# giolucasd/ssrl-vit-mae-jepa

Measured on AMD Instinct MI355X. Metric: images/sec pretrain step (fwd+bwd+opt), ViT-S/8 96px MAE, 1/2/4/8 MI355X, higher is better.
Workload: dtype bf16; 1 GPU; ViT-S/8 96px MAE (enc 384x12x6h, dec 192x2x6h, mask_ratio 0.75), batch 2000/GPU, full step; global_batch=2000, per_gpu_batch=2000, parallelism=dp1

## Files before the change

ssrl_vit_mae_jepa_amd/csrc/engine.hip:

```cpp
#include <string>
#include <vector>
#include <cmath>
#include <cstring>
#include <cstdlib>
#include <cstdint>
#include "kernels.h"

namespace mae {

static thread_local char g_err[1024] = "";
void set_error(const char* fmt, ...) {
  va_list ap;
  va_start(ap, fmt);
  vsnprintf(g_err, sizeof(g_err), fmt, ap);
  va_end(ap);
}
int hip_fail(hipError_t err, const char* what, const char* file, int line) {
  set_error("HIP error %d (%s) at %s:%d: %s", (int)err, hipGetErrorString(err), file, line, what);
  return 2;
}

struct ParamInfo {
  std::string name;
  int64_t offset = 0, numel = 0;
// ... 14 lines not shown
struct TimerSlot {
  std::vector<std::pair<hipEvent_t, hipEvent_t>> ev;
  size_t used = 0;
  double flops = 0, bytes = 0;
};

}

using namespace mae;

struct mae_engine {
  mae_config_t cfg;
  int act = MAE_F32;
  int D, depth, H, Dd, dd, Hd, P, L, G, C, img, p, mlp;
  int PO;
  std::vector<ParamInfo> params;
  int64_t arena_elems = 0, trainable_elems = 0, trans_elems = 0;
  int i_enc_mask, i_cls, i_pos, i_patch_w, i_patch_b, i_norm_w, i_norm_b;
  int i_dec_mask, i_dec_pos, i_de_w, i_de_b, i_dn_w, i_dn_b, i_pred_w, i_pred_b;
  std::vector<BlockRefs> enc, dec;
  bool timers_on = false;
  TimerSlot timers[TK_COUNT];
  PartialsTable ln_tab;
};

namespace mae {

static int add_param(mae_engine* e, const std::string& name, std::initializer_list<int64_t> shape, int flags) {
  ParamInfo pi;
  pi.name = name;
  pi.ndim = (int)shape.size();
  pi.numel = 1;
  int i = 0;
  for (int64_t s : shape) { pi.shape[i++] = s; pi.numel *= s; }
  pi.flags = flags;
  e->params.push_back(pi);
  return (int)e->params.size() - 1;
}

static BlockRefs add_block(mae_engine* e, const std::string& pfx, int d, int mlp) {
  const int T = MAE_PARAM_TRAINABLE, M = MAE_PARAM_TRAINABLE | MAE_PARAM_MATRIX;
  BlockRefs r;
  r.ln1_w = add_param(e, pfx + ".norm1.weight", {d}, T);
  r.ln1_b = add_param(e, pfx + ".norm1.bias", {d}, T);
  r.qkv_w = add_param(e, pfx + ".attn.qkv.weight", {3 * (int64_t)d, d}, M);
  r.qkv_b = add_param(e, pfx + ".attn.qkv.bias", {3 * (int64_t)d}, T);
// ... 2 lines not shown
  r.ln2_w = add_param(e, pfx + ".norm2.weight", {d}, T);
  r.ln2_b = add_param(e, pfx + ".norm2.bias", {d}, T);
  r.fc1_w = add_param(e, pfx + ".mlp.fc1.weight", {(int64_t)mlp * d, d}, M);
  r.fc1_b = add_param(e, pfx + ".mlp.fc1.bias", {(int64_t)mlp * d}, T);
  r.fc2_w = add_param(e, pfx + ".mlp.fc2.weight", {d, (int64_t)mlp * d}, M);
  r.fc2_b = add_param(e, pfx + ".mlp.fc2.bias", {d}, T);
  return r;
}

struct LayerBufs {
  int64_t x_mid, ln1, mean1, rstd1, qkv, lse, att, ln2, mean2, rstd2, fc1_pre, fc1_act;
};

struct Plan {
  int B, k, m;
  int dec_B, dec_T;
  int64_t Me, Md, Mp;
  int64_t keep32, mask32, inv, pred_rows;
  int64_t patchA;
  std::vector<int64_t> enc_x, dec_x;
  std::vector<LayerBufs> enc, dec;
  int64_t enc_norm, enc_mean, enc_rstd, xdec, dec_norm, dec_mean, dec_rstd, pred;
  int64_t branch_a, branch_b;
  int64_t dpred, d_decn, dres, dres_c, d_ln, d_att, d_qkv, d_hidden, d_xdec, dtok;
  int64_t ln_partial, ln_partial_stride, split_partial, wgrad_scratch, loss_scratch;
  int64_t total;
};

static Plan make_plan_ex(const mae_engine* e, int B, int k, int dec_B, int dec_T, int m_seq) {
  Plan pl;
  pl.B = B; pl.k = k; pl.m = m_seq;
  pl.dec_B = dec_B; pl.dec_T = dec_T;
  pl.Me = (int64_t)B * k; pl.Md = (int64_t)dec_B * dec_T; pl.Mp = (int64_t)dec_B * m_seq;
  const int64_t as = (int64_t)dtype_size(e->act);
  int64_t off = 0;
  auto take = [&](int64_t bytes) { const int64_t o = off; off += round_up(std::max<int64_t>(bytes, 4), 256); return o; };
  pl.keep32 = take(pl.Me * 4);
  pl.mask32 = take(pl.Mp * 4);
  pl.inv = take(pl.Md * 4);
  pl.pred_rows = take(pl.Mp * 4);
  pl.patchA = take(pl.Me * e->P * as);
  auto layers = [&](int n, int64_t M, int d, int heads, int T, std::vector<int64_t>& xs, std::vector<LayerBufs>& ls) {
    const int64_t seqs = M / std::max(T, 1);
    xs.resize(n + 1);
    ls.resize(n);
    xs[0] = take(M * d * 4);
    for (int i = 0; i < n; ++i) {
// ... 3 lines not shown
      b.lse = take(seqs * heads * T * 4);
      b.att = take(M * d * as);
      b.x_mid = take(M * d * 4);
      b.ln2 = take(M * d * as); b.mean2 = take(M * 4); b.rstd2 = take(M * 4);
      b.fc1_pre = take(M * e->mlp * d * as);
      b.fc1_act = take(M * e->mlp * d * as);
      xs[i + 1] = take(M * d * 4);
    }
  };
  layers(e->depth, pl.Me, e->D, e->H, k, pl.enc_x, pl.enc);
  pl.enc_norm = take(pl.Me * e->D * as); pl.enc_mean = take(pl.Me * 4); pl.enc_rstd = take(pl.Me * 4);
  pl.xdec = take(pl.Me * e->Dd * as);
  layers(e->dd, pl.Md, e->Dd, e->Hd, dec_T, pl.dec_x, pl.dec);
  pl.dec_norm = take(std::max<int64_t>(pl.Mp, 1) * e->Dd * as);
  pl.dec_mean = take(std::max<int64_t>(pl.Mp, 1) * 4); pl.dec_rstd = take(std::max<int64_t>(pl.Mp, 1) * 4);
  pl.pred = take(std::max<int64_t>(pl.Mp, 1) * e->PO * 4);
  const int64_t R = std::max(pl.Me * e->D, pl.Md * e->Dd);
  pl.branch_a = take(R * as);
  pl.branch_b = take(R * as);
  pl.dpred = take(std::max<int64_t>(pl.Mp, 1) * e->PO * as);
  pl.d_decn = take(std::max<int64_t>(pl.Mp, 1) * e->Dd * as);
  pl.dres = take(R * 4);
  pl.dres_c = take(R * as);
  pl.d_ln = take(R * as);
  pl.d_att = take(R * as);
  pl.d_qkv = take(3 * R * as);
  pl.d_hidden = take((int64_t)e->mlp * R * as);
  pl.d_xdec = take(pl.Me * e->Dd * as);
  pl.dtok = take(pl.Me * e->D * as);
  const int maxd = std::max(e->D, e->Dd);
  pl.ln_partial_stride = (int64_t)2 * LN_BWD_MAX_BLOCKS * maxd * 4;
  pl.ln_partial = take(pl.ln_partial_stride * std::min(2 * (e->depth + e->dd) + 2, (int)PartialsTable::MAX));
  pl.split_partial = take((int64_t)512 * maxd * 4);
  int64_t wg = 0;
  auto wgs = [&](int64_t M, int N, int K) { wg = std::max(wg, linear_wgrad_scratch_bytes(M, N, K)); };
  wgs(pl.Me, 3 * e->D, e->D); wgs(pl.Me, e->mlp * e->D, e->D); wgs(pl.Me, e->D, e->mlp * e->D); wgs(pl.Me, e->D, e->D);
  wgs(pl.Md, 3 * e->Dd, e->Dd); wgs(pl.Md, e->mlp * e->Dd, e->Dd); wgs(pl.Md, e->Dd, e->mlp * e->Dd); wgs(pl.Md, e->Dd, e->Dd);
  wgs(pl.Me, e->D, e->P); wgs(pl.Me, e->Dd, e->D); wgs(std::max<int64_t>(pl.Mp, 1), e->PO, e->Dd);
  auto wgp = [&](int64_t M, int d) {
    wg = std::max(wg, linear_wgrad_pair_scratch_bytes(M, d, e->mlp * d, e->mlp * d, d));
    wg = std::max(wg, linear_wgrad_pair_scratch_bytes(M, d, d, 3 * d, d));
  };
  wgp(pl.Me, e->D); wgp(pl.Md, e->Dd);
  pl.wgrad_scratch = take(wg);
  pl.loss_scratch = take(4096 * 4);
  pl.total = off;
// ... 58 lines not shown
  const int64_t side = mode == MAE_EPI_RESID ? 4 : (mode == MAE_EPI_MUL || mode == MAE_EPI_DGELU) ? os : 0;
  return (double)(M * K * as + (int64_t)N * K * as + M * N * (outs * os + side));
}

static int linear(const Ctx& c, const void* A, int wi, int bi, int64_t M, int N, int K, int mode, int out_dt, void* out, void* out2,
                  const void* aux) {
  mae_engine* e = c.e; hipStream_t s = c.s;
  Epi ep; ep.mode = mode; ep.bias = bi >= 0 ? c.P(bi) : nullptr; ep.aux = aux; ep.out = out; ep.out2 = out2; ep.out_dt = out_dt;
  RUN(TK_LINEAR, 2.0 * M * N * K, gemm_bytes(M, N, K, c.as, (int64_t)dtype_size(out_dt), mode), launch_linear_fwd(A, c.W(wi), M, N, K, c.act, ep, s));
  return 0;
}

static int dgrad(const Ctx& c, const void* dY, int wi, int64_t M, int N, int K, int mode, void* out, const void* aux) {
  mae_engine* e = c.e; hipStream_t s = c.s;
  Epi ep; ep.mode = mode; ep.aux = aux; ep.out = out; ep.out_dt = c.act;
  if (c.act == MAE_BF16) {
    RUN(TK_LINEAR, 2.0 * M * N * K, gemm_bytes(M, K, N, 2, 2, mode), launch_linear_fwd(dY, c.WT(wi), M, K, N, MAE_BF16, ep, s));
  } else {
    RUN(TK_LINEAR, 2.0 * M * N * K, gemm_bytes(M, K, N, 4, 4, mode), launch_linear_dgrad(dY, c.W(wi), M, N, K, MAE_F32, ep, s));
  }
  return 0;
}

static int wgrad(const Ctx& c, const Plan& pl, const void* dY, const void* A, int64_t M, int N, int K, int wi, int bi) {
  mae_engine* e = c.e; hipStream_t s = c.s;
  RUN(TK_WGRAD, 2.0 * M * N * K, (double)(M * (N + K) * c.as + (int64_t)N * K * 4),
      launch_linear_wgrad(dY, A, M, N, K, c.act, c.Gp(wi), bi >= 0 ? c.Gp(bi) : nullptr, c.buf<>(pl.wgrad_scratch), s));
  return 0;
}

static int wgrad_pair(const Ctx& c, const Plan& pl, int64_t M, const void* dY0, const void* A0, int N0, int K0, int w0, int b0,
                      const void* dY1, const void* A1, int N1, int K1, int w1, int b1) {
  mae_engine* e = c.e;
  hipStream_t s = c.s;
  RUN(TK_WGRAD, 2.0 * M * ((double)N0 * K0 + (double)N1 * K1),
      (double)(M * (int64_t)(N0 + K0 + N1 + K1) * c.as + ((int64_t)N0 * K0 + (int64_t)N1 * K1) * 4),
      launch_linear_wgrad_pair(dY0, A0, N0, K0, c.Gp(w0), c.Gp(b0), dY1, A1, N1, K1, c.Gp(w1), c.Gp(b1), M, c.act, c.buf<>(pl.wgrad_scratch), s));
  return 0;
}

static int ln_fwd(const Ctx& c, const float* x, const void* branch, float* x_sum, const int32_t* row_map, const float* gamma,
                  const float* beta, float eps, int64_t rows, int d, int y_dt, void* y, float* mean, float* rstd,
                  const float* image_scale = nullptr, int T = 0) {
  mae_engine* e = c.e; hipStream_t s = c.s;
  const int64_t ys = (int64_t)dtype_size(y_dt);
  RUN(TK_LN_FWD, 0, rows * d * (branch ? 8 + 2 * ys : 4 + ys),
      launch_layernorm_fwd(x, branch, x_sum, row_map, gamma, beta, eps, rows, d, y_dt, y, mean, rstd, s, image_scale, T));
  return 0;
}

static int ln_bwd(const Ctx& c, const Plan& pl, const void* dy, const float* x, const int32_t* row_map, int wi, int bi, const float* mean,
                  const float* rstd, int64_t rows, int d, int accumulate, const float* copy_scale = nullptr, int T = 0) {
  mae_engine* e = c.e; hipStream_t s = c.s;
  float* slot = c.buf<float>(pl.ln_partial + (int64_t)(e->ln_tab.n % PartialsTable::MAX) * pl.ln_partial_stride);
  RUN(TK_LN_BWD, 0, rows * d * (12 + 2 * c.as),
      launch_layernorm_bwd(dy, c.act, x, row_map, c.P(wi), mean, rstd, rows, d, accumulate, c.buf<float>(pl.dres), c.buf<>(pl.dres_c),
                           c.Gp(wi), c.Gp(bi), slot, s, &e->ln_tab, copy_scale, T));
  return 0;
}

static int block_forward(const Ctx& c, const Plan& pl, const BlockRefs& r, const LayerBufs& b, int64_t M, int d, int heads, int Bn, int T,
                         int64_t x_prev, bool add_prev, int64_t x_in, const float* scale_prev = nullptr, const float* scale_att = nullptr) {
  mae_engine* e = c.e; hipStream_t s = c.s;
  const int hd = d / heads, hid = e->mlp * d;
  const float eps = 1e-6f;
  MAE_TRY(ln_fwd(c, c.buf<float>(add_prev ? x_prev : x_in), add_prev ? c.buf<>(pl.branch_b) : nullptr, add_prev ? c.buf<float>(x_in) : nullptr,
                 nullptr, c.P(r.ln1_w), c.P(r.ln1_b), eps, M, d, c.act, c.buf<>(b.ln1), c.buf<float>(b.mean1), c.buf<float>(b.rstd1),
                 add_prev ? scale_prev : nullptr, T));
  MAE_TRY(linear(c, c.buf<>(b.ln1), r.qkv_w, r.qkv_b, M, 3 * d, d, MAE_EPI_NONE, c.act, c.buf<>(b.qkv), nullptr, nullptr));
  RUN(TK_ATTN_FWD, 4.0 * Bn * heads * (double)T * T * hd, M * 4 * d * c.as, launch_attention_fwd(c.buf<>(b.qkv), Bn, T, heads, hd, c.act, c.buf<>(b.att), c.buf<float>(b.lse), s));
  MAE_TRY(linear(c, c.buf<>(b.att), r.proj_w, r.proj_b, M, d, d, MAE_EPI_NONE, c.act, c.buf<>(pl.branch_a), nullptr, nullptr));
  MAE_TRY(ln_fwd(c, c.buf<float>(x_in), c.buf<>(pl.branch_a), c.buf<float>(b.x_mid), nullptr, c.P(r.ln2_w), c.P(r.ln2_b), eps, M, d, c.act,
                 c.buf<>(b.ln2), c.buf<float>(b.mean2), c.buf<float>(b.rstd2), scale_att, T));
  if (c.fwd_only)
    MAE_TRY(linear(c, c.buf<>(b.ln2), r.fc1_w, r.fc1_b, M, hid, d, MAE_EPI_GELU_ACT, c.act, c.buf<>(b.fc1_act), nullptr, nullptr));
  else
    MAE_TRY(linear(c, c.buf<>(b.ln2), r.fc1_w, r.fc1_b, M, hid, d, MAE_EPI_GELU_GRAD, c.act, c.buf<>(b.fc1_pre), c.buf<>(b.fc1_act), nullptr));
  MAE_TRY(linear(c, c.buf<>(b.fc1_act), r.fc2_w, r.fc2_b, M, d, hid, MAE_EPI_NONE, c.act, c.buf<>(pl.branch_b), nullptr, nullptr));
  return 0;
}

static int block_backward(const Ctx& c, const Plan& pl, const BlockRefs& r, const LayerBufs& b, int64_t M, int d, int heads, int Bn, int T,
                          int64_t x_in, const float* scale_prev = nullptr, const float* scale_att = nullptr) {
  mae_engine* e = c.e; hipStream_t s = c.s;
  const int hd = d / heads, hid = e->mlp * d;
  void* dres_c = c.buf<>(pl.dres_c);
  MAE_TRY(dgrad(c, dres_c, r.fc2_w, M, d, hid, MAE_EPI_MUL, c.buf<>(pl.d_hidden), c.buf<>(b.fc1_pre)));
  MAE_TRY(wgrad_pair(c, pl, M, dres_c, c.buf<>(b.fc1_act), d, hid, r.fc2_w, r.fc2_b, c.buf<>(pl.d_hidden), c.buf<>(b.ln2), hid, d, r.fc1_w, r.fc1_b));
  MAE_TRY(dgrad(c, c.buf<>(pl.d_hidden), r.fc1_w, M, hid, d, MAE_EPI_NONE, c.buf<>(pl.d_ln), nullptr));
  MAE_TRY(ln_bwd(c, pl, c.buf<>(pl.d_ln), c.buf<float>(b.x_mid), nullptr, r.ln2_w, r.ln2_b, c.buf<float>(b.mean2), c.buf<float>(b.rstd2), M, d, 1, scale_att, T));
  MAE_TRY(dgrad(c, dres_c, r.proj_w, M, d, d, MAE_EPI_NONE, c.buf<>(pl.d_att), nullptr));
  RUN(TK_ATTN_BWD, 10.0 * Bn * heads * (double)T * T * hd, M * 9 * d * c.as, launch_attention_bwd(c.buf<>(b.qkv), c.buf<>(b.att), c.buf<>(pl.d_att), c.buf<float>(b.lse), Bn, T, heads, hd, c.act, c.buf<>(pl.d_qkv), s));
  MAE_TRY(wgrad_pair(c, pl, M, dres_c, c.buf<>(b.att), d, d, r.proj_w, r.proj_b, c.buf<>(pl.d_qkv), c.buf<>(b.ln1), 3 * d, d, r.qkv_w, r.qkv_b));
  MAE_TRY(dgrad(c, c.buf<>(pl.d_qkv), r.qkv_w, M, 3 * d, d, MAE_EPI_NONE, c.buf<>(pl.d_ln), nullptr));
  MAE_TRY(ln_bwd(c, pl, c.buf<>(pl.d_ln), c.buf<float>(x_in), nullptr, r.ln1_w, r.ln1_b, c.buf<float>(b.mean1), c.buf<float>(b.rstd1), M, d, 1, scale_prev, T));
  return 0;
}

static bool batch_in_bound(const mae_engine* e, int B) {
  return (int64_t)B * e->L * std::max(3 * e->D, e->mlp * std::max(e->D, e->Dd)) < (1ll << 40);
}

static int check_common(const mae_engine* e, const void* params, const void* wcache, int B, const void* ws, const char* who) {
  MAE_REQUIRE(e, "%s: null engine", who);
  MAE_REQUIRE(params && ws, "%s: null params/workspace", who);
  MAE_REQUIRE(e->act == MAE_F32 || wcache, "%s: bf16 engine needs the weight cache", who);
  MAE_REQUIRE(batch_in_bound(e, B), "%s: batch too large", who);
  MAE_REQUIRE(((uintptr_t)ws & 255) == 0 && ((uintptr_t)params & 15) == 0, "%s: workspace must be 256-byte aligned, params 16-byte", who);
  return 0;
}

static int check_call(const mae_engine* e, const void* params, const void* wcache, int B, int k, const void* ws, int64_t ws_bytes,
                      Plan* pl, const char* who) {
  MAE_TRY(check_common(e, params, wcache, B, ws, who));
  MAE_REQUIRE(B > 0 && k >= 1 && k <= e->L, "%s: batch %d / num_keep %d out of range (L = %d)", who, B, k, e->L);
  *pl = make_plan(e, B, k);
  MAE_REQUIRE(ws_bytes >= pl->total, "%s: workspace too small (%lld < %lld bytes)", who, (long long)ws_bytes, (long long)pl->total);
// ... 39 lines not shown
static int forward_decoder_impl(const Ctx& c, const Plan& pl, float* x_pred_out, const JepaSeq* jp = nullptr) {
  mae_engine* e = c.e; hipStream_t s = c.s;
  MAE_REQUIRE(pl.m > 0, "forward_decoder: nothing is masked (num_keep == sequence_length)");
  MAE_TRY(linear(c, c.buf<>(pl.enc_norm), e->i_de_w, e->i_de_b, pl.Me, e->Dd, e->D, MAE_EPI_NONE, c.act, c.buf<>(pl.xdec), nullptr, nullptr));
  if (jp) {
    MAE_TRY(launch_build_tail_row_map(pl.dec_B, pl.dec_T, pl.m, c.buf<int32_t>(pl.pred_rows), s));
    RUN(TK_DATA, 0, pl.Md * e->Dd * 4 + pl.Me * e->Dd * c.as, launch_predictor_assemble(c.buf<>(pl.xdec), c.act, jp->ctx32, jp->tgt32, c.P(e->i_dec_mask), c.P(e->i_dec_pos), pl.B, pl.k, jp->nblk, pl.m, e->L, e->Dd, c.buf<float>(pl.dec_x[0]), s));
  } else {
    MAE_TRY(launch_build_inverse(c.buf<int32_t>(pl.keep32), pl.B, pl.k, e->L, c.buf<int32_t>(pl.inv), s));
    MAE_TRY(launch_build_row_map(c.buf<int32_t>(pl.mask32), pl.B, pl.m, e->L, c.buf<int32_t>(pl.pred_rows), s));
    RUN(TK_DATA, 0, pl.Md * e->Dd * 4 + pl.Me * e->Dd * c.as, launch_decoder_assemble(c.buf<>(pl.xdec), c.act, c.buf<int32_t>(pl.inv), c.P(e->i_dec_mask), c.P(e->i_dec_pos), pl.B, pl.k, e->L, e->Dd, c.buf<float>(pl.dec_x[0]), s));
  }
  for (int i = 0; i < e->dd; ++i)
    MAE_TRY(block_forward(c, pl, e->dec[i], pl.dec[i], pl.Md, e->Dd, e->Hd, pl.dec_B, pl.dec_T, i ? pl.dec[i - 1].x_mid : 0, i > 0, pl.dec_x[i]));
  MAE_TRY(ln_fwd(c, c.buf<float>(pl.dec[e->dd - 1].x_mid), c.buf<>(pl.branch_b), c.buf<float>(pl.dec_x[e->dd]), c.buf<int32_t>(pl.pred_rows),
                 c.P(e->i_dn_w), c.P(e->i_dn_b), 1e-6f, pl.Mp, e->Dd, c.act, c.buf<>(pl.dec_norm), c.buf<float>(pl.dec_mean), c.buf<float>(pl.dec_rstd)));
  MAE_TRY(linear(c, c.buf<>(pl.dec_norm), e->i_pred_w, e->i_pred_b, pl.Mp, e->PO, e->Dd, MAE_EPI_NONE, MAE_F32, x_pred_out ? (void*)x_pred_out : c.buf<>(pl.pred), nullptr, nullptr));
  return 0;
}

static int reach_point(const Ctx& c, int j) {
  mae_engine* e = c.e; hipStream_t s = c.s;
  if (!c.ready || !c.ready[j]) return 0;
  if (e->ln_tab.n > 0) {
    RUN(TK_LN_BWD, 0, 0, launch_sum_partials_many(e->ln_tab, s));
    e->ln_tab.n = 0;
  }
  MAE_HIP(hipEventRecord((hipEvent_t)c.ready[j], s));
  return 0;
}

static void backward_begin(const Ctx& c) { c.e->ln_tab.n = 0; }
static int backward_end(const Ctx& c) {
  mae_engine* e = c.e; hipStream_t s = c.s;
  if (e->ln_tab.n > 0) RUN(TK_LN_BWD, 0, 0, launch_sum_partials_many(e->ln_tab, s));
  e->ln_tab.n = 0;
  return 0;
}

static int backward_decoder_impl(const Ctx& c, const Plan& pl, const JepaSeq* jp = nullptr) {
  mae_engine* e = c.e; hipStream_t s = c.s;
  float* dres = c.buf<float>(pl.dres);
  MAE_TRY(wgrad(c, pl, c.buf<>(pl.dpred), c.buf<>(pl.dec_norm), pl.Mp, e->PO, e->Dd, e->i_pred_w, e->i_pred_b));
  MAE_TRY(dgrad(c, c.buf<>(pl.dpred), e->i_pred_w, pl.Mp, e->PO, e->Dd, MAE_EPI_NONE, c.buf<>(pl.d_decn), nullptr));
  RUN(TK_DATA, 0, (pl.Md - pl.Mp) * e->Dd * (4 + c.as), launch_zero_unpredicted_rows(jp ? nullptr : c.buf<int32_t>(pl.inv), pl.Md, pl.dec_T, pl.m, e->Dd, c.act, dres, c.buf<>(pl.dres_c), s));
  MAE_TRY(ln_bwd(c, pl, c.buf<>(pl.d_decn), c.buf<float>(pl.dec_x[e->dd]), c.buf<int32_t>(pl.pred_rows), e->i_dn_w, e->i_dn_b, c.buf<float>(pl.dec_mean),
                 c.buf<float>(pl.dec_rstd), pl.Mp, e->Dd, 0));
  for (int i = e->dd - 1; i >= 0; --i)
    MAE_TRY(block_backward(c, pl, e->dec[i], pl.dec[i], pl.Md, e->Dd, e->Hd, pl.dec_B, pl.dec_T, pl.dec_x[i]));
  if (jp)
    RUN(TK_DATA, 0, pl.Md * e->Dd * 4 + pl.Me * e->Dd * c.as, launch_predictor_assemble_bwd(dres, pl.B, pl.k, jp->nblk, pl.m, e->Dd, c.act, c.buf<>(pl.d_xdec), c.Gp(e->i_dec_mask), c.buf<float>(pl.split_partial), s));
  else
    RUN(TK_DATA, 0, pl.Md * e->Dd * 4 + pl.Me * e->Dd * c.as, launch_decoder_assemble_bwd(dres, c.buf<int32_t>(pl.inv), c.buf<int32_t>(pl.keep32), pl.B, pl.k, e->L, e->Dd, c.act, c.buf<>(pl.d_xdec), c.Gp(e->i_dec_mask), c.buf<float>(pl.split_partial), s));
  MAE_TRY(wgrad(c, pl, c.buf<>(pl.d_xdec), c.buf<>(pl.enc_norm), pl.Me, e->Dd, e->D, e->i_de_w, e->i_de_b));
  MAE_TRY(dgrad(c, c.buf<>(pl.d_xdec), e->i_de_w, pl.Me, e->Dd, e->D, MAE_EPI_NONE, c.buf<>(pl.d_ln), nullptr));
  return reach_point(c, 0);
}

static int backward_encoder_impl(const Ctx& c, const Plan& pl) {
  mae_engine* e = c.e; hipStream_t s = c.s;
  MAE_TRY(ln_bwd(c, pl, c.buf<>(pl.d_ln), c.buf<float>(pl.enc_x[e->depth]), nullptr, e->i_norm_w, e->i_norm_b, c.buf<float>(pl.enc_mean),
                 c.buf<float>(pl.enc_rstd), pl.Me, e->D, 0));
  for (int i = e->depth - 1; i >= 0; --i) {
    MAE_TRY(block_backward(c, pl, e->enc[i], pl.enc[i], pl.Me, e->D, e->H, pl.B, pl.k, pl.enc_x[i]));
    if (i > 0) MAE_TRY(reach_point(c, e->depth - i));
  }
  RUN(TK_DATA, 0, pl.Me * e->D * (4 + c.as), launch_visible_grad_split(c.buf<float>(pl.dres), c.buf<int32_t>(pl.keep32), pl.Me, e->D, c.act, c.buf<>(pl.dtok), c.Gp(e->i_cls), c.buf<float>(pl.split_partial), s));
  MAE_TRY(wgrad(c, pl, c.buf<>(pl.dtok), c.buf<>(pl.patchA), pl.Me, e->D, e->P, e->i_patch_w, e->i_patch_b));
  return 0;
}

static int backward_impl(const Ctx& c, const Plan& pl, const float* d_x_encoded_extra = nullptr, const JepaSeq* jp = nullptr) {
  mae_engine* e = c.e; hipStream_t s = c.s;
  backward_begin(c);
  MAE_TRY(backward_decoder_impl(c, pl, jp));
  if (d_x_encoded_extra) MAE_TRY(launch_add_into(d_x_encoded_extra, c.buf<>(pl.d_ln), c.act, pl.Me * e->D, s));
  MAE_TRY(backward_encoder_impl(c, pl));
  MAE_TRY(backward_end(c));
  if (c.ready && c.ready[e->depth]) MAE_HIP(hipEventRecord((hipEvent_t)c.ready[e->depth], s));
  return 0;
}

}

extern "C" const char* mae_last_error(void) { return mae::g_err; }
extern "C" int mae_abi_version(void) { return MAE_ABI_VERSION; }

extern "C" int mae_engine_create(const mae_config_t* cfg, mae_engine_t** out) {
  MAE_REQUIRE(cfg && out, "mae_engine_create: null argument");
  MAE_REQUIRE(cfg->image_size > 0 && cfg->patch_size > 0 && cfg->image_size % cfg->patch_size == 0,
              "image_size %d must be a positive multiple of patch_size %d", cfg->image_size, cfg->patch_size);
  MAE_REQUIRE(cfg->in_chans > 0 && cfg->embed_dim > 0 && cfg->depth > 0 && cfg->decoder_embed_dim > 0 && cfg->decoder_depth > 0,
              "mae_engine_create: non-positive model dimension");
  MAE_REQUIRE(cfg->num_heads > 0 && cfg->embed_dim % cfg->num_heads == 0, "dim should be divisible by num_heads (%d %% %d)", cfg->embed_dim, cfg->num_heads);
  MAE_REQUIRE(cfg->decoder_num_heads > 0 && cfg->decoder_embed_dim % cfg->decoder_num_heads == 0,
              "decoder dim should be divisible by decoder_num_heads (%d %% %d)", cfg->decoder_embed_dim, cfg->decoder_num_heads);
  MAE_REQUIRE(cfg->embed_dim % 4 == 0 && cfg->decoder_embed_dim % 4 == 0 && cfg->embed_dim <= 1024 && cfg->decoder_embed_dim <= 1024,
// ... 33 lines not shown
  e->i_dn_w = add_param(e, "decoder.decoder_norm.weight", {e->Dd}, T);
  e->i_dn_b = add_param(e, "decoder.decoder_norm.bias", {e->Dd}, T);
  e->i_pred_w = add_param(e, "decoder.decoder_pred.weight", {e->PO, e->Dd}, M);
  e->i_pred_b = add_param(e, "decoder.decoder_pred.bias", {e->PO}, T);
  int64_t off = 0, toff = 0;
  for (auto& pi : e->params)
    if (pi.flags & MAE_PARAM_TRAINABLE) {
      pi.offset = off; off += round_up(pi.numel, 64);
      if (pi.flags & MAE_PARAM_MATRIX) { pi.t_off = toff; toff += round_up(pi.numel, 64); }
    }
  e->trainable_elems = off;
  for (auto& pi : e->params)
    if (!(pi.flags & MAE_PARAM_TRAINABLE)) { pi.offset = off; off += round_up(pi.numel, 64); }
  e->arena_elems = off;
  e->trans_elems = toff;
  *out = e;
  return 0;
}

extern "C" void mae_engine_destroy(mae_engine_t* e) {
  if (!e) return;
  for (auto& t : e->timers)
    for (auto& pr : t.ev) { (void)hipEventDestroy(pr.first); (void)hipEventDestroy(pr.second); }
  delete e;
}

extern "C" int64_t mae_engine_num_params(const mae_engine_t* e) { return e ? (int64_t)e->params.size() : 0; }
extern "C" int64_t mae_engine_arena_elems(const mae_engine_t* e) { return e ? e->arena_elems : 0; }
extern "C" int64_t mae_engine_trainable_elems(const mae_engine_t* e) { return e ? e->trainable_elems : 0; }

extern "C" int mae_engine_param_info(const mae_engine_t* e, int64_t index, const char** name, int64_t* offset, int64_t* numel,
                                     int32_t* ndim, int64_t shape[4], int32_t* flags) {
  MAE_REQUIRE(e && index >= 0 && index < (int64_t)e->params.size(), "mae_engine_param_info: index out of range");
  const ParamInfo& pi = e->params[index];
  if (name) *name = pi.name.c_str();
  if (offset) *offset = pi.offset;
  if (numel) *numel = pi.numel;
  if (ndim) *ndim = pi.ndim;
  if (shape) for (int i = 0; i < 4; ++i) shape[i] = pi.shape[i];
  if (flags) *flags = pi.flags;
  return 0;
}

extern "C" int64_t mae_engine_workspace_bytes(const mae_engine_t* e, int32_t batch, int32_t num_keep) {
  if (!e || batch <= 0 || num_keep < 1 || num_keep > e->L) return -1;
  return make_plan(e, batch, num_keep).total;
// ... 99 lines not shown
extern "C" int mae_engine_backward(mae_engine_t* e, const float* params, const void* wcache, const float* d_pred,
                                   const float* d_x_encoded_extra, int32_t batch, int32_t num_keep, int32_t num_mask,
                                   void* workspace, int64_t workspace_bytes, float* grads, void* stream) {
  Plan pl;
  MAE_TRY(check_call(e, params, wcache, batch, num_keep, workspace, workspace_bytes, &pl, "mae_engine_backward"));
  MAE_REQUIRE(d_pred && grads, "mae_engine_backward: null d_pred/grads");
  MAE_REQUIRE(num_mask == pl.m && pl.m > 0, "mae_engine_backward: num_mask mismatch");
  Ctx c = make_ctx(e, params, wcache, grads, workspace, stream);
  hipStream_t s = c.s;
  MAE_TRY(launch_cast(d_pred, MAE_F32, c.buf<>(pl.dpred), e->act, pl.Mp * e->PO, s));
  return backward_impl(c, pl, d_x_encoded_extra);
}

extern "C" int mae_engine_backward_decoder(mae_engine_t* e, const float* params, const void* wcache, const float* d_pred,
                                           int32_t batch, int32_t num_keep, int32_t num_mask, void* workspace,
                                           int64_t workspace_bytes, float* grads, float* d_x_encoded, void* stream) {
  Plan pl;
  MAE_TRY(check_call(e, params, wcache, batch, num_keep, workspace, workspace_bytes, &pl, "mae_engine_backward_decoder"));
  MAE_REQUIRE(d_pred && grads, "mae_engine_backward_decoder: null d_pred/grads");
  MAE_REQUIRE(num_mask == pl.m && pl.m > 0, "mae_engine_backward_decoder: num_mask mismatch");
  Ctx c = make_ctx(e, params, wcache, grads, workspace, stream);
  hipStream_t s = c.s;
  MAE_TRY(launch_cast(d_pred, MAE_F32, c.buf<>(pl.dpred), e->act, pl.Mp * e->PO, s));
  backward_begin(c);
  MAE_TRY(backward_decoder_impl(c, pl));
  MAE_TRY(backward_end(c));
  if (d_x_encoded) MAE_TRY(launch_cast(c.buf<>(pl.d_ln), e->act, d_x_encoded, MAE_F32, pl.Me * e->D, s));
  return 0;
}

extern "C" int mae_engine_backward_encoder(mae_engine_t* e, const float* params, const void* wcache, const float* d_x_encoded,
                                           int32_t batch, int32_t num_keep, void* workspace, int64_t workspace_bytes,
                                           float* grads, void* stream) {
  Plan pl;
  MAE_TRY(check_call(e, params, wcache, batch, num_keep, workspace, workspace_bytes, &pl, "mae_engine_backward_encoder"));
  MAE_REQUIRE(d_x_encoded && grads, "mae_engine_backward_encoder: null d_x_encoded/grads");
  Ctx c = make_ctx(e, params, wcache, grads, workspace, stream);
  hipStream_t s = c.s;
  MAE_TRY(launch_cast(d_x_encoded, MAE_F32, c.buf<>(pl.d_ln), e->act, pl.Me * e->D, s));
  backward_begin(c);
  MAE_TRY(backward_encoder_impl(c, pl));
  return backward_end(c);
}

extern "C" int64_t mae_engine_encoder_grad_elems(const mae_engine_t* e) { return e ? e->params[e->i_dec_mask].offset : 0; }

extern "C" int mae_engine_decoder_decode(mae_engine_t* e, const float* params, const void* wcache, const float* x, int32_t batch,
                                         void* workspace, int64_t workspace_bytes, float* out, void* stream) {
  Plan pl;
  MAE_TRY(check_call(e, params, wcache, batch, 1, workspace, workspace_bytes, &pl, "mae_engine_decoder_decode"));
  MAE_REQUIRE(x && out, "mae_engine_decoder_decode: null x/out");
  Ctx c = make_ctx(e, params, wcache, nullptr, workspace, stream);
  hipStream_t s = c.s;
  MAE_TRY(launch_add_rows_pos(x, c.P(e->i_dec_pos), pl.Md, e->L, e->Dd, c.buf<float>(pl.dec_x[0]), s));
  for (int i = 0; i < e->dd; ++i)
    MAE_TRY(block_forward(c, pl, e->dec[i], pl.dec[i], pl.Md, e->Dd, e->Hd, pl.B, e->L, i ? pl.dec[i - 1].x_mid : 0, i > 0, pl.dec_x[i]));
  float* stat = c.buf<float>(pl.dres);
  MAE_TRY(ln_fwd(c, c.buf<float>(pl.dec[e->dd - 1].x_mid), c.buf<>(pl.branch_b), c.buf<float>(pl.dec_x[e->dd]), nullptr, c.P(e->i_dn_w),
                 c.P(e->i_dn_b), 1e-6f, pl.Md, e->Dd, c.act, c.buf<>(pl.d_ln), stat, stat + pl.Md));
  return ln_fwd(c, c.buf<float>(pl.dec_x[e->dd]), nullptr, nullptr, nullptr, c.P(e->i_dn_w), c.P(e->i_dn_b), 1e-6f, pl.Md, e->Dd, MAE_F32, out,
                stat, stat + pl.Md);
}

// ... 313 lines not shown
  MAE_TRY(forward_encoder_impl(c, pl, images, image_dtype, nullptr));
  const bool cls = pool == MAE_POOL_CLS;
  const bool range = !with_cls || pool == MAE_POOL_MEAN_PATCHES;
  const int lo = with_cls ? 1 : 0;
  void* dfeat = enc_bwd ? (cls ? c.buf<>(cp.dpooled) : c.buf<>(pl.d_ln)) : nullptr;
  if (range) {
    RUN(TK_LOSS, 2.0 * B * C * D * (train ? 2 : 1), (double)B * (L - lo) * D * c.as + (double)C * D * 4 + (enc_bwd ? (double)pl.Me * D * c.as : 0.0),
        launch_classifier_head_range(c.buf<>(pl.enc_norm), e->act, B, L, D, lo, L, head, head + (int64_t)C * D, C, labels, grad_scale, logits,
                                     c.buf<float>(cp.row_loss), c.buf<int32_t>(cp.row_correct), loss_out, correct_out,
                                     train ? c.buf<float>(cp.pooled) : nullptr, train ? c.buf<float>(cp.dlogits) : nullptr, dfeat, s, soft));
  } else {
    RUN(TK_LOSS, 2.0 * B * C * D * (train ? 2 : 1), (cls ? (double)B * D : (double)pl.Me * D) * c.as + (double)C * D * 4 + (enc_bwd && !cls ? (double)pl.Me * D * c.as : 0.0),
        launch_classifier_head(c.buf<>(pl.enc_norm), e->act, B, L, D, pool, head, head + (int64_t)C * D, C, labels, grad_scale, logits,
                               c.buf<float>(cp.row_loss), c.buf<int32_t>(cp.row_correct), loss_out, correct_out,
                               train ? c.buf<float>(cp.pooled) : nullptr, train ? c.buf<float>(cp.dlogits) : nullptr, dfeat,
                               c.buf<float>(pl.enc_mean), c.buf<float>(pl.enc_rstd), c.buf<float>(cp.mean_c), c.buf<float>(cp.rstd_c),
                               enc_bwd && cls ? c.buf<int32_t>(cp.cls_rows) : nullptr, s, soft));
  }
  if (!train) return 0;
  RUN(TK_WGRAD, 2.0 * B * C * D, (double)B * (C + D) * 4, launch_classifier_head_wgrad(c.buf<float>(cp.dlogits), c.buf<float>(cp.pooled), B, C, D,
                                                                                    c.buf<float>(cp.head_partial), c.buf<float>(cp.head_sum), head_grads, s));
  if (!enc_bwd) return 0;
  float* dres = c.buf<float>(pl.dres);
  backward_begin(c);
  if (cls) {
    RUN(TK_DATA, 0, (pl.Me - B) * D * (4 + c.as), launch_zero_token_rows(pl.Me, L, D, e->act, dres, c.buf<>(pl.dres_c), s));
    MAE_TRY(ln_bwd(c, pl, c.buf<>(cp.dpooled), c.buf<float>(pl.enc_x[e->depth]), c.buf<int32_t>(cp.cls_rows), e->i_norm_w, e->i_norm_b,
                   c.buf<float>(cp.mean_c), c.buf<float>(cp.rstd_c), B, D, 0, c.scale_row(2 * e->depth - 1, B), L));
  } else {
    MAE_TRY(ln_bwd(c, pl, c.buf<>(pl.d_ln), c.buf<float>(pl.enc_x[e->depth]), nullptr, e->i_norm_w, e->i_norm_b, c.buf<float>(pl.enc_mean),
                   c.buf<float>(pl.enc_rstd), pl.Me, D, 0, c.scale_row(2 * e->depth - 1, B), L));
  }
  for (int i = e->depth - 1; i >= e->depth - train_blocks; --i)
    MAE_TRY(block_backward(c, pl, e->enc[i], pl.enc[i], pl.Me, D, e->H, B, L, pl.enc_x[i], i ? c.scale_row(2 * i - 1, B) : nullptr,
                           c.scale_row(2 * i, B)));
  if (train_embed) {
    if (with_cls)
      RUN(TK_DATA, 0, pl.Me * D * (4 + c.as), launch_full_grad_split(dres, B, L, D, e->act, c.buf<>(pl.dtok), pos_grad, c.Gp(e->i_cls), c.buf<float>(cp.pos_partial), s));
    else
      RUN(TK_DATA, 0, pl.Me * D * (4 + c.as), launch_patch_grad_split(dres, B, L, D, e->act, c.buf<>(pl.dtok), pos_grad, c.Gp(e->i_cls), c.buf<float>(cp.pos_partial), s));
    MAE_TRY(wgrad(c, pl, c.buf<>(pl.dtok), c.buf<>(pl.patchA), pl.Me, D, e->P, e->i_patch_w, e->i_patch_b));
  }
  return backward_end(c);
}

}

extern "C" int64_t mae_engine_classifier_workspace_bytes(const mae_engine_t* e, int32_t batch, int32_t num_classes) {
  if (!e || batch <= 0 || num_classes < 2 || num_classes > HEAD_MAX_CLASSES) return -1;
// ... 181 lines not shown
```

ssrl_vit_mae_jepa_amd/csrc/k_layernorm.hip:

```cpp
#include "kernels.h"

#ifndef MAE_LN_NT
#define MAE_LN_NT 5
#endif
#if MAE_LN_NT & 1
#define LN_ST_A store4_nt
#else
#define LN_ST_A store4
#endif
#if MAE_LN_NT & 2
#define LN_ST_B store4_nt
#else
#define LN_ST_B store4
#endif
#if MAE_LN_NT & 4
#define LN_LD load4_nt
#else
#define LN_LD load4
#endif

namespace mae {

template <int LPR>
__device__ __forceinline__ float group_sum(float v) {
// ... 89 lines not shown
  MAE_REQUIRE(!image_scale || (branch && rows_per_image > 0), "layernorm_fwd: an image scale needs a branch and rows_per_image > 0");
  MAE_REQUIRE(dim % 4 == 0 && dim >= 4 && dim <= 1024, "layernorm: dim %d must be a multiple of 4 in [4, 1024]", dim);
  const int lpr = ln_lanes_per_row(dim / 4), nv = (int)cdiv(dim / 4, lpr);
  const int grid = (int)std::min<int64_t>(cdiv(rows, 4 * (64 / lpr)), 256 * 32);
#define LN(T, NV, ADD, LPR) hipLaunchKernelGGL((layernorm_fwd_kernel<T, NV, ADD, LPR>), dim3(grid), dim3(256), 0, s, x, (const T*)branch, x_out, row_map, gamma, beta, eps, rows, dim, (T*)y, mean, rstd)
#define LN_NV(T, ADD, LPR) switch (nv) { case 1: LN(T, 1, ADD, LPR); break; case 2: LN(T, 2, ADD, LPR); break; case 3: LN(T, 3, ADD, LPR); break; default: LN(T, 4, ADD, LPR); }
#define LN_LPR(T, ADD) switch (lpr) { case 16: LN_NV(T, ADD, 16) break; case 32: LN_NV(T, ADD, 32) break; default: LN_NV(T, ADD, 64) }
#define LNS(T, NV, LPR) hipLaunchKernelGGL((layernorm_fwd_kernel<T, NV, true, LPR, const float*, int>), dim3(grid), dim3(256), 0, s, x, (const T*)branch, x_out, row_map, gamma, beta, eps, rows, dim, (T*)y, mean, rstd, image_scale, rows_per_image)
#define LNS_NV(T, LPR) switch (nv) { case 1: LNS(T, 1, LPR); break; case 2: LNS(T, 2, LPR); break; case 3: LNS(T, 3, LPR); break; default: LNS(T, 4, LPR); }
#define LNS_LPR(T) switch (lpr) { case 16: LNS_NV(T, 16) break; case 32: LNS_NV(T, 32) break; default: LNS_NV(T, 64) }
  if (image_scale) { if (y_dt == MAE_BF16) { LNS_LPR(bf16) } else { LNS_LPR(float) } }
  else if (y_dt == MAE_BF16) { if (branch) { LN_LPR(bf16, true) } else { LN_LPR(bf16, false) } }
  else { if (branch) { LN_LPR(float, true) } else { LN_LPR(float, false) } }
#undef LNS_LPR
#undef LNS_NV
#undef LNS
#undef LN_LPR
#undef LN_NV
#undef LN
  MAE_LAUNCH_CHECK();
  return 0;
}

template <class T, int NV, int LPR, class... S>
__global__ void __launch_bounds__(256) layernorm_bwd_kernel(const T* __restrict__ dy, const float* __restrict__ x,
                                                            const int32_t* __restrict__ row_map,
                                                            const float* __restrict__ gamma, const float* __restrict__ mean,
                                                            const float* __restrict__ rstd, int64_t rows, int dim,
                                                            int accumulate, float* __restrict__ dx_io, T* __restrict__ dx_copy,
                                                            float* __restrict__ partial, S... scale_args) {
  constexpr bool SCALE = sizeof...(S) != 0;
  constexpr int RPW = 64 / LPR;
  extern __shared__ __attribute__((aligned(16))) float red[];
  const int lane = threadIdx.x & 63, wave = threadIdx.x >> 6, li = lane & (LPR - 1), sub = lane / LPR;
  const int D4 = dim >> 2;
  const float inv_d = 1.0f / (float)dim;
  f32x4 gam[NV], dg[NV], db[NV];
#pragma unroll
  for (int i = 0; i < NV; ++i) {
    const int c = li + LPR * i;
    gam[i] = (c < D4) ? load4(gamma + c * 4) : f32x4{0.f, 0.f, 0.f, 0.f};
    dg[i] = f32x4{0.f, 0.f, 0.f, 0.f};
    db[i] = f32x4{0.f, 0.f, 0.f, 0.f};
  }
  for (int64_t r0 = (blockIdx.x * 4ll + wave) * RPW; r0 < rows; r0 += (int64_t)gridDim.x * 4 * RPW) {
    const bool live = r0 + sub < rows;
// ... 14 lines not shown
        if (live) {
          dg[i] += d * xh[i];
          db[i] += d;
        }
        s1 += g[i][0] + g[i][1] + g[i][2] + g[i][3];
        s2 += g[i][0] * xh[i][0] + g[i][1] * xh[i][1] + g[i][2] * xh[i][2] + g[i][3] * xh[i][3];
      }
    }
    s1 = group_sum<LPR>(s1) * inv_d;
    s2 = group_sum<LPR>(s2) * inv_d;
#pragma unroll
    for (int i = 0; i < NV; ++i) {
      const int c = li + LPR * i;
      if (c < D4 && live) {
        f32x4 d = (g[i] - s1 - xh[i] * s2) * rs;
        float* pd = dx_io + src * dim + c * 4;
        if (accumulate) d += load4(pd);
        LN_ST_A(pd, d);
        if (SCALE) LN_ST_B(dx_copy + src * dim + c * 4, d * sc);
        else if (dx_copy) LN_ST_B(dx_copy + src * dim + c * 4, d);
      }
    }
  }
#pragma unroll
  for (int i = 0; i < NV; ++i) {
    const int c = li + LPR * i;
    if (c < D4) {
      store4(red + ((wave * RPW + sub) * 2 + 0) * dim + c * 4, dg[i]);
      store4(red + ((wave * RPW + sub) * 2 + 1) * dim + c * 4, db[i]);
    }
  }
  __syncthreads();
  for (int c = threadIdx.x; c < 2 * dim; c += 256) {
    float v = 0.f;
#pragma unroll
    for (int gidx = 0; gidx < 4 * RPW; ++gidx) v += red[gidx * 2 * dim + c];
    partial[(int64_t)blockIdx.x * 2 * dim + c] = v;
  }
}

int launch_layernorm_bwd(const void* dy, int dy_dt, const float* x, const int32_t* row_map, const float* gamma,
                         const float* mean, const float* rstd, int64_t rows, int dim, int accumulate, float* dx_io,
                         void* dx_copy, float* dgamma, float* dbeta, float* partial, hipStream_t s, PartialsTable* defer,
                         const float* copy_scale, int rows_per_image) {
  MAE_REQUIRE(dy && x && gamma && mean && rstd && dx_io && dgamma && dbeta && partial && rows > 0, "layernorm_bwd: null buffer");
  MAE_REQUIRE(!copy_scale || (dx_copy && rows_per_image > 0), "layernorm_bwd: a copy scale needs dx_copy and rows_per_image > 0");
  MAE_REQUIRE(dim % 4 == 0 && dim >= 4 && dim <= 1024, "layernorm: dim %d must be a multiple of 4 in [4, 1024]", dim);
  if (defer && defer->n == PartialsTable::MAX) {
    MAE_TRY(launch_sum_partials_many(*defer, s));
    defer->n = 0;
  }
  const int lpr = ln_lanes_per_row(dim / 4), nv = (int)cdiv(dim / 4, lpr);
  const int grid = (int)std::min<int64_t>(cdiv(rows, 4 * (64 / lpr)), LN_BWD_MAX_BLOCKS);
  const size_t lds = (size_t)8 * (64 / lpr) * dim * sizeof(float);
#define LNB(T, NV, LPR) hipLaunchKernelGGL((layernorm_bwd_kernel<T, NV, LPR>), dim3(grid), dim3(256), lds, s, (const T*)dy, x, row_map, gamma, mean, rstd, rows, dim, accumulate, dx_io, (T*)dx_copy, partial)
#define LNB_NV(T, LPR) switch (nv) { case 1: LNB(T, 1, LPR); break; case 2: LNB(T, 2, LPR); break; case 3: LNB(T, 3, LPR); break; default: LNB(T, 4, LPR); }
#define LNB_LPR(T) switch (lpr) { case 16: LNB_NV(T, 16) break; case 32: LNB_NV(T, 32) break; default: LNB_NV(T, 64) }
#define LNBS(T, NV, LPR) hipLaunchKernelGGL((layernorm_bwd_kernel<T, NV, LPR, const float*, int>), dim3(grid), dim3(256), lds, s, (const T*)dy, x, row_map, gamma, mean, rstd, rows, dim, accumulate, dx_io, (T*)dx_copy, partial, copy_scale, rows_per_image)
#define LNBS_NV(T, LPR) switch (nv) { case 1: LNBS(T, 1, LPR); break; case 2: LNBS(T, 2, LPR); break; case 3: LNBS(T, 3, LPR); break; default: LNBS(T, 4, LPR); }
#define LNBS_LPR(T) switch (lpr) { case 16: LNBS_NV(T, 16) break; case 32: LNBS_NV(T, 32) break; default: LNBS_NV(T, 64) }
  if (copy_scale) { if (dy_dt == MAE_BF16) { LNBS_LPR(bf16) } else { LNBS_LPR(float) } }
  else if (dy_dt == MAE_BF16) { LNB_LPR(bf16) } else { LNB_LPR(float) }
#undef LNBS_LPR
#undef LNBS_NV
#undef LNBS
#undef LNB_LPR
#undef LNB_NV
#undef LNB
  MAE_LAUNCH_CHECK();
  if (defer) {
    const int i = defer->n++;
    if (i == 0) defer->block_begin[0] = 0;
    defer->partial[i] = partial; defer->out0[i] = dgamma; defer->out1[i] = dbeta;
    defer->G[i] = grid; defer->C[i] = 2 * dim; defer->split[i] = dim;
    defer->block_begin[i + 1] = defer->block_begin[i] + (int)cdiv(2 * dim, 32);
    return 0;
  }
// ... 45 lines not shown
```

Baseline: 93940 images/s.

## Overlap backward weight-gradient pairs on a side stream and shrink LN-bwd LDS

```diff
diff --git a/ssrl_vit_mae_jepa_amd/csrc/engine.hip b/ssrl_vit_mae_jepa_amd/csrc/engine.hip
--- a/ssrl_vit_mae_jepa_amd/csrc/engine.hip
+++ b/ssrl_vit_mae_jepa_amd/csrc/engine.hip
@@ -60,6 +60,12 @@
   bool timers_on = false;
   TimerSlot timers[TK_COUNT];
   PartialsTable ln_tab;
+  hipStream_t side = nullptr;
+  int side_dev = -1;
+  hipEvent_t ev_fork = nullptr, ev_done = nullptr;
+  bool overlap = false;
+  bool side_pending = false;
+  int dres_sel = 0;
 };
 
 namespace mae {
@@ -108,7 +114,7 @@
   std::vector<LayerBufs> enc, dec;
   int64_t enc_norm, enc_mean, enc_rstd, xdec, dec_norm, dec_mean, dec_rstd, pred;
   int64_t branch_a, branch_b;
-  int64_t dpred, d_decn, dres, dres_c, d_ln, d_att, d_qkv, d_hidden, d_xdec, dtok;
+  int64_t dpred, d_decn, dres, dres_c, dres_c2, d_ln, d_att, d_qkv, d_hidden, d_xdec, dtok;
   int64_t ln_partial, ln_partial_stride, split_partial, wgrad_scratch, loss_scratch;
   int64_t total;
 };
@@ -158,6 +164,7 @@
   pl.d_decn = take(std::max<int64_t>(pl.Mp, 1) * e->Dd * as);
   pl.dres = take(R * 4);
   pl.dres_c = take(R * as);
+  pl.dres_c2 = take(R * as);
   pl.d_ln = take(R * as);
   pl.d_att = take(R * as);
   pl.d_qkv = take(3 * R * as);
@@ -262,8 +269,19 @@
   return 0;
 }
 
+static int join_side(const Ctx& c) {
+  mae_engine* e = c.e;
+  if (!e->side_pending) return 0;
+  MAE_HIP(hipStreamWaitEvent(c.s, e->ev_done, 0));
+  e->side_pending = false;
+  return 0;
+}
+
+static void* cur_dres_c(const Ctx& c, const Plan& pl) { return c.buf<>(c.e->dres_sel ? pl.dres_c2 : pl.dres_c); }
+
 static int wgrad(const Ctx& c, const Plan& pl, const void* dY, const void* A, int64_t M, int N, int K, int wi, int bi) {
   mae_engine* e = c.e; hipStream_t s = c.s;
+  MAE_TRY(join_side(c));
   RUN(TK_WGRAD, 2.0 * M * N * K, (double)(M * (N + K) * c.as + (int64_t)N * K * 4),
       launch_linear_wgrad(dY, A, M, N, K, c.act, c.Gp(wi), bi >= 0 ? c.Gp(bi) : nullptr, c.buf<>(pl.wgrad_scratch), s));
   return 0;
@@ -273,9 +291,19 @@
                       const void* dY1, const void* A1, int N1, int K1, int w1, int b1) {
   mae_engine* e = c.e;
   hipStream_t s = c.s;
+  if (e->overlap) {
+    MAE_TRY(join_side(c));
+    MAE_HIP(hipEventRecord(e->ev_fork, c.s));
+    MAE_HIP(hipStreamWaitEvent(e->side, e->ev_fork, 0));
+    s = e->side;
+  }
   RUN(TK_WGRAD, 2.0 * M * ((double)N0 * K0 + (double)N1 * K1),
       (double)(M * (int64_t)(N0 + K0 + N1 + K1) * c.as + ((int64_t)N0 * K0 + (int64_t)N1 * K1) * 4),
       launch_linear_wgrad_pair(dY0, A0, N0, K0, c.Gp(w0), c.Gp(b0), dY1, A1, N1, K1, c.Gp(w1), c.Gp(b1), M, c.act, c.buf<>(pl.wgrad_scratch), s));
+  if (e->overlap) {
+    MAE_HIP(hipEventRecord(e->ev_done, e->side));
+    e->side_pending = true;
+  }
   return 0;
 }
 
@@ -294,7 +322,7 @@
   mae_engine* e = c.e; hipStream_t s = c.s;
   float* slot = c.buf<float>(pl.ln_partial + (int64_t)(e->ln_tab.n % PartialsTable::MAX) * pl.ln_partial_stride);
   RUN(TK_LN_BWD, 0, rows * d * (12 + 2 * c.as),
-      launch_layernorm_bwd(dy, c.act, x, row_map, c.P(wi), mean, rstd, rows, d, accumulate, c.buf<float>(pl.dres), c.buf<>(pl.dres_c),
+      launch_layernorm_bwd(dy, c.act, x, row_map, c.P(wi), mean, rstd, rows, d, accumulate, c.buf<float>(pl.dres), cur_dres_c(c, pl),
                            c.Gp(wi), c.Gp(bi), slot, s, &e->ln_tab, copy_scale, T));
   return 0;
 }
@@ -324,15 +352,21 @@
                           int64_t x_in, const float* scale_prev = nullptr, const float* scale_att = nullptr) {
   mae_engine* e = c.e; hipStream_t s = c.s;
   const int hd = d / heads, hid = e->mlp * d;
-  void* dres_c = c.buf<>(pl.dres_c);
+  const bool ov = e->overlap;
+  void* dres_c = cur_dres_c(c, pl);
   MAE_TRY(dgrad(c, dres_c, r.fc2_w, M, d, hid, MAE_EPI_MUL, c.buf<>(pl.d_hidden), c.buf<>(b.fc1_pre)));
+  if (ov) MAE_TRY(dgrad(c, c.buf<>(pl.d_hidden), r.fc1_w, M, hid, d, MAE_EPI_NONE, c.buf<>(pl.d_ln), nullptr));
   MAE_TRY(wgrad_pair(c, pl, M, dres_c, c.buf<>(b.fc1_act), d, hid, r.fc2_w, r.fc2_b, c.buf<>(pl.d_hidden), c.buf<>(b.ln2), hid, d, r.fc1_w, r.fc1_b));
-  MAE_TRY(dgrad(c, c.buf<>(pl.d_hidden), r.fc1_w, M, hid, d, MAE_EPI_NONE, c.buf<>(pl.d_ln), nullptr));
+  if (!ov) MAE_TRY(dgrad(c, c.buf<>(pl.d_hidden), r.fc1_w, M, hid, d, MAE_EPI_NONE, c.buf<>(pl.d_ln), nullptr));
+  if (ov) e->dres_sel ^= 1;
   MAE_TRY(ln_bwd(c, pl, c.buf<>(pl.d_ln), c.buf<float>(b.x_mid), nullptr, r.ln2_w, r.ln2_b, c.buf<float>(b.mean2), c.buf<float>(b.rstd2), M, d, 1, scale_att, T));
+  dres_c = cur_dres_c(c, pl);
   MAE_TRY(dgrad(c, dres_c, r.proj_w, M, d, d, MAE_EPI_NONE, c.buf<>(pl.d_att), nullptr));
   RUN(TK_ATTN_BWD, 10.0 * Bn * heads * (double)T * T * hd, M * 9 * d * c.as, launch_attention_bwd(c.buf<>(b.qkv), c.buf<>(b.att), c.buf<>(pl.d_att), c.buf<float>(b.lse), Bn, T, heads, hd, c.act, c.buf<>(pl.d_qkv), s));
+  if (ov) MAE_TRY(dgrad(c, c.buf<>(pl.d_qkv), r.qkv_w, M, 3 * d, d, MAE_EPI_NONE, c.buf<>(pl.d_ln), nullptr));
   MAE_TRY(wgrad_pair(c, pl, M, dres_c, c.buf<>(b.att), d, d, r.proj_w, r.proj_b, c.buf<>(pl.d_qkv), c.buf<>(b.ln1), 3 * d, d, r.qkv_w, r.qkv_b));
-  MAE_TRY(dgrad(c, c.buf<>(pl.d_qkv), r.qkv_w, M, 3 * d, d, MAE_EPI_NONE, c.buf<>(pl.d_ln), nullptr));
+  if (!ov) MAE_TRY(dgrad(c, c.buf<>(pl.d_qkv), r.qkv_w, M, 3 * d, d, MAE_EPI_NONE, c.buf<>(pl.d_ln), nullptr));
+  if (ov) e->dres_sel ^= 1;
   MAE_TRY(ln_bwd(c, pl, c.buf<>(pl.d_ln), c.buf<float>(x_in), nullptr, r.ln1_w, r.ln1_b, c.buf<float>(b.mean1), c.buf<float>(b.rstd1), M, d, 1, scale_prev, T));
   return 0;
 }
@@ -418,6 +452,7 @@
 static int reach_point(const Ctx& c, int j) {
   mae_engine* e = c.e; hipStream_t s = c.s;
   if (!c.ready || !c.ready[j]) return 0;
+  MAE_TRY(join_side(c));
   if (e->ln_tab.n > 0) {
     RUN(TK_LN_BWD, 0, 0, launch_sum_partials_many(e->ln_tab, s));
     e->ln_tab.n = 0;
@@ -426,9 +461,42 @@
   return 0;
 }
 
-static void backward_begin(const Ctx& c) { c.e->ln_tab.n = 0; }
+static bool bwd_overlap_sel() {
+  const char* v = getenv("MAE_BWD_OVERLAP");
+  return v && v[0] == '1' && !v[1];
+}
+static int side_stream_ready(mae_engine* e) {
+  int dev = 0;
+  MAE_HIP(hipGetDevice(&dev));
+  if (e->side && e->side_dev == dev) return 0;
+  if (e->side) {
+    (void)hipStreamDestroy(e->side); (void)hipEventDestroy(e->ev_fork); (void)hipEventDestroy(e->ev_done);
+    e->side = nullptr; e->ev_fork = e->ev_done = nullptr;
+  }
+  hipStream_t st = nullptr;
+  hipEvent_t a = nullptr, b = nullptr;
+  MAE_HIP(hipStreamCreateWithFlags(&st, hipStreamNonBlocking));
+  if (hipEventCreateWithFlags(&a, hipEventDisableTiming) != hipSuccess || hipEventCreateWithFlags(&b, hipEventDisableTiming) != hipSuccess) {
+    if (a) (void)hipEventDestroy(a);
+    (void)hipStreamDestroy(st);
+    MAE_REQUIRE(false, "backward overlap: cannot create the fork / join events");
+  }
+  e->side = st; e->ev_fork = a; e->ev_done = b; e->side_dev = dev;
+  return 0;
+}
+
+static int backward_begin(const Ctx& c) {
+  mae_engine* e = c.e;
+  e->ln_tab.n = 0;
+  e->dres_sel = 0;
+  e->side_pending = false;
+  e->overlap = bwd_overlap_sel();
+  if (e->overlap) MAE_TRY(side_stream_ready(e));
+  return 0;
+}
 static int backward_end(const Ctx& c) {
   mae_engine* e = c.e; hipStream_t s = c.s;
+  MAE_TRY(join_side(c));
   if (e->ln_tab.n > 0) RUN(TK_LN_BWD, 0, 0, launch_sum_partials_many(e->ln_tab, s));
   e->ln_tab.n = 0;
   return 0;
@@ -439,7 +507,7 @@
   float* dres = c.buf<float>(pl.dres);
   MAE_TRY(wgrad(c, pl, c.buf<>(pl.dpred), c.buf<>(pl.dec_norm), pl.Mp, e->PO, e->Dd, e->i_pred_w, e->i_pred_b));
   MAE_TRY(dgrad(c, c.buf<>(pl.dpred), e->i_pred_w, pl.Mp, e->PO, e->Dd, MAE_EPI_NONE, c.buf<>(pl.d_decn), nullptr));
-  RUN(TK_DATA, 0, (pl.Md - pl.Mp) * e->Dd * (4 + c.as), launch_zero_unpredicted_rows(jp ? nullptr : c.buf<int32_t>(pl.inv), pl.Md, pl.dec_T, pl.m, e->Dd, c.act, dres, c.buf<>(pl.dres_c), s));
+  RUN(TK_DATA, 0, (pl.Md - pl.Mp) * e->Dd * (4 + c.as), launch_zero_unpredicted_rows(jp ? nullptr : c.buf<int32_t>(pl.inv), pl.Md, pl.dec_T, pl.m, e->Dd, c.act, dres, cur_dres_c(c, pl), s));
   MAE_TRY(ln_bwd(c, pl, c.buf<>(pl.d_decn), c.buf<float>(pl.dec_x[e->dd]), c.buf<int32_t>(pl.pred_rows), e->i_dn_w, e->i_dn_b, c.buf<float>(pl.dec_mean),
                  c.buf<float>(pl.dec_rstd), pl.Mp, e->Dd, 0));
   for (int i = e->dd - 1; i >= 0; --i)
@@ -468,7 +536,7 @@
 
 static int backward_impl(const Ctx& c, const Plan& pl, const float* d_x_encoded_extra = nullptr, const JepaSeq* jp = nullptr) {
   mae_engine* e = c.e; hipStream_t s = c.s;
-  backward_begin(c);
+  MAE_TRY(backward_begin(c));
   MAE_TRY(backward_decoder_impl(c, pl, jp));
   if (d_x_encoded_extra) MAE_TRY(launch_add_into(d_x_encoded_extra, c.buf<>(pl.d_ln), c.act, pl.Me * e->D, s));
   MAE_TRY(backward_encoder_impl(c, pl));
@@ -548,6 +616,7 @@
   if (!e) return;
   for (auto& t : e->timers)
     for (auto& pr : t.ev) { (void)hipEventDestroy(pr.first); (void)hipEventDestroy(pr.second); }
+  if (e->side) { (void)hipStreamDestroy(e->side); (void)hipEventDestroy(e->ev_fork); (void)hipEventDestroy(e->ev_done); }
   delete e;
 }
 
@@ -693,7 +762,7 @@
   Ctx c = make_ctx(e, params, wcache, grads, workspace, stream);
   hipStream_t s = c.s;
   MAE_TRY(launch_cast(d_pred, MAE_F32, c.buf<>(pl.dpred), e->act, pl.Mp * e->PO, s));
-  backward_begin(c);
+  MAE_TRY(backward_begin(c));
   MAE_TRY(backward_decoder_impl(c, pl));
   MAE_TRY(backward_end(c));
   if (d_x_encoded) MAE_TRY(launch_cast(c.buf<>(pl.d_ln), e->act, d_x_encoded, MAE_F32, pl.Me * e->D, s));
@@ -709,7 +778,7 @@
   Ctx c = make_ctx(e, params, wcache, grads, workspace, stream);
   hipStream_t s = c.s;
   MAE_TRY(launch_cast(d_x_encoded, MAE_F32, c.buf<>(pl.d_ln), e->act, pl.Me * e->D, s));
-  backward_begin(c);
+  MAE_TRY(backward_begin(c));
   MAE_TRY(backward_encoder_impl(c, pl));
   return backward_end(c);
 }
@@ -1069,9 +1138,9 @@
                                                                                     c.buf<float>(cp.head_partial), c.buf<float>(cp.head_sum), head_grads, s));
   if (!enc_bwd) return 0;
   float* dres = c.buf<float>(pl.dres);
-  backward_begin(c);
+  MAE_TRY(backward_begin(c));
   if (cls) {
-    RUN(TK_DATA, 0, (pl.Me - B) * D * (4 + c.as), launch_zero_token_rows(pl.Me, L, D, e->act, dres, c.buf<>(pl.dres_c), s));
+    RUN(TK_DATA, 0, (pl.Me - B) * D * (4 + c.as), launch_zero_token_rows(pl.Me, L, D, e->act, dres, cur_dres_c(c, pl), s));
     MAE_TRY(ln_bwd(c, pl, c.buf<>(cp.dpooled), c.buf<float>(pl.enc_x[e->depth]), c.buf<int32_t>(cp.cls_rows), e->i_norm_w, e->i_norm_b,
                    c.buf<float>(cp.mean_c), c.buf<float>(cp.rstd_c), B, D, 0, c.scale_row(2 * e->depth - 1, B), L));
   } else {
diff --git a/ssrl_vit_mae_jepa_amd/csrc/k_layernorm.hip b/ssrl_vit_mae_jepa_amd/csrc/k_layernorm.hip
--- a/ssrl_vit_mae_jepa_amd/csrc/k_layernorm.hip
+++ b/ssrl_vit_mae_jepa_amd/csrc/k_layernorm.hip
@@ -135,6 +135,8 @@
   return 0;
 }
 
+__host__ __device__ constexpr int ln_bwd_slots(int lpr, int nv) { return 4 * (64 / lpr) / (nv <= 3 ? 2 : 4); }
+
 template <class T, int NV, int LPR, class... S>
 __global__ void __launch_bounds__(256) layernorm_bwd_kernel(const T* __restrict__ dy, const float* __restrict__ x,
                                                             const int32_t* __restrict__ row_map,
@@ -195,20 +197,39 @@
       }
     }
   }
-#pragma unroll
-  for (int i = 0; i < NV; ++i) {
-    const int c = li + LPR * i;
-    if (c < D4) {
-      store4(red + ((wave * RPW + sub) * 2 + 0) * dim + c * 4, dg[i]);
-      store4(red + ((wave * RPW + sub) * 2 + 1) * dim + c * 4, db[i]);
-    }
-  }
-  __syncthreads();
-  for (int c = threadIdx.x; c < 2 * dim; c += 256) {
-    float v = 0.f;
-#pragma unroll
-    for (int gidx = 0; gidx < 4 * RPW; ++gidx) v += red[gidx * 2 * dim + c];
-    partial[(int64_t)blockIdx.x * 2 * dim + c] = v;
+  constexpr int G = 4 * RPW, SLOTS = ln_bwd_slots(LPR, NV);
+  constexpr int NC = (8 * LPR * NV + 255) / 256;
+  const int grp = wave * RPW + sub;
+  float colsum[NC];
+#pragma unroll
+  for (int j = 0; j < NC; ++j) colsum[j] = 0.f;
+#pragma unroll
+  for (int g0 = 0; g0 < G; g0 += SLOTS) {
+    if (g0 > 0) __syncthreads();
+    if (grp >= g0 && grp < g0 + SLOTS) {
+#pragma unroll
+      for (int i = 0; i < NV; ++i) {
+        const int c = li + LPR * i;
+        if (c < D4) {
+          store4(red + ((grp - g0) * 2 + 0) * dim + c * 4, dg[i]);
+          store4(red + ((grp - g0) * 2 + 1) * dim + c * 4, db[i]);
+        }
+      }
+    }
+    __syncthreads();
+#pragma unroll
+    for (int j = 0; j < NC; ++j) {
+      const int c = threadIdx.x + 256 * j;
+      if (c < 2 * dim) {
+#pragma unroll
+        for (int k = 0; k < SLOTS; ++k) colsum[j] += red[k * 2 * dim + c];
+      }
+    }
+  }
+#pragma unroll
+  for (int j = 0; j < NC; ++j) {
+    const int c = threadIdx.x + 256 * j;
+    if (c < 2 * dim) partial[(int64_t)blockIdx.x * 2 * dim + c] = colsum[j];
   }
 }
 
@@ -225,7 +246,7 @@
   }
   const int lpr = ln_lanes_per_row(dim / 4), nv = (int)cdiv(dim / 4, lpr);
   const int grid = (int)std::min<int64_t>(cdiv(rows, 4 * (64 / lpr)), LN_BWD_MAX_BLOCKS);
-  const size_t lds = (size_t)8 * (64 / lpr) * dim * sizeof(float);
+  const size_t lds = (size_t)ln_bwd_slots(lpr, nv) * 2 * dim * sizeof(float);
 #define LNB(T, NV, LPR) hipLaunchKernelGGL((layernorm_bwd_kernel<T, NV, LPR>), dim3(grid), dim3(256), lds, s, (const T*)dy, x, row_map, gamma, mean, rstd, rows, dim, accumulate, dx_io, (T*)dx_copy, partial)
 #define LNB_NV(T, LPR) switch (nv) { case 1: LNB(T, 1, LPR); break; case 2: LNB(T, 2, LPR); break; case 3: LNB(T, 3, LPR); break; default: LNB(T, 4, LPR); }
 #define LNB_LPR(T) switch (lpr) { case 16: LNB_NV(T, 16) break; case 32: LNB_NV(T, 32) break; default: LNB_NV(T, 64) }
```

New measurement: 93830 images/s. Within noise of the previous version (-0.1%).
